# ISU-PAAL/DeepDFA

Measured on AMD Instinct MI355X. Metric: train_graphs_per_sec, higher is better.
Workload: dtype bf16; 1 GPU; model=DeepDFA-FlowGNN-GGNN(n_steps=5,D=128), global_batch=256, avg_nodes_per_graph=45, parallelism=dp1

## Files before the change

csrc/bindings.hip:

```cpp

#include <torch/extension.h>

#include <hip/hip_runtime.h>
#include <hip/hip_bf16.h>
#include <c10/hip/HIPStream.h>
#include <c10/util/accumulate.h>

#include <climits>

template <typename T>
void launch_embed4_fwd(const T*, const long*, T*, int, int, hipStream_t);
template <typename T, typename TO>
void launch_embed4_fwd2(const T*, const long*, TO*, int, int, hipStream_t);
template <typename T>
void launch_embed4_bwd(const T*, const long*, float*, long, int, hipStream_t);
template <typename T>
void launch_spmm_sum(const int*, const int*, const T*, T*, int, int, hipStream_t);
template <typename T>
void launch_gru_gates_fwd(const T*, const T*, const T*, T*, T*, T*, T*, long, int, hipStream_t);
template <typename T>
void launch_gru_gates_bwd(const T*, const T*, const T*, const T*, const T*, const T*, T*, T*, T*,
                          long, int, hipStream_t);
template <typename T>
void launch_attn_pool_fwd(const T*, const T*, const int*, T*, float*, int, int, hipStream_t);
template <typename T>
void launch_attn_pool_bwd(const T*, const T*, const float*, const int*, T*, T*, float*, int, int,
                          hipStream_t);
void launch_segment_max(const float*, const int*, float*, int, hipStream_t);
template <typename T>
void launch_gru_gates2_fwd(const T*, const T*, T*, T*, T*, T*, T*, long, int, hipStream_t);
template <typename T>
void launch_gru_gates2_bwd(const T*, const T*, const T*, const T*, const T*, const T*, T*, T*,
                           long, int, hipStream_t);
template <typename T>
void launch_colsum(const T*, float*, int, int, hipStream_t);
template <typename T>
void launch_spmm_sum_strided(const int*, const int*, const T*, T*, int, int, long,
                             hipStream_t);
void launch_gemm_bias2(const __hip_bfloat16*, const __hip_bfloat16*, const __hip_bfloat16*,
                       const __hip_bfloat16*, const __hip_bfloat16*, long,
                       const __hip_bfloat16*, long, __hip_bfloat16*, int, int, int, int,
                       hipStream_t, const int* = nullptr, const int* = nullptr, long = 0,
                       __hip_bfloat16* = nullptr);
bool launch_gates_gemm(const __hip_bfloat16*, const __hip_bfloat16*, const __hip_bfloat16*,
                       const __hip_bfloat16*, const __hip_bfloat16*, const __hip_bfloat16*,
                       const __hip_bfloat16*, __hip_bfloat16*, __hip_bfloat16*,
                       __hip_bfloat16*, int, int, hipStream_t);
void launch_gemm_bias(const __hip_bfloat16*, const __hip_bfloat16*, const __hip_bfloat16*,
                      const __hip_bfloat16*, const __hip_bfloat16*, __hip_bfloat16*, int, int,
                      int, int, hipStream_t);
void launch_wgrad(const __hip_bfloat16*, const __hip_bfloat16*, const __hip_bfloat16*, float*,
                  float*, int, int, int, int, hipStream_t, float* = nullptr,
                  float* = nullptr, float* = nullptr, float* = nullptr);
template <typename T>
void launch_layernorm_fwd(const T*, const float*, const float*, T*, float*, float*, long, int,
                          float, hipStream_t);
template <typename T>
void launch_layernorm_bwd(const T*, const T*, const float*, const float*, const float*, T*, long,
                          int, hipStream_t);
template <typename T>
void launch_layernorm_wgrad(const T*, const T*, const float*, const float*, float*, float*, long,
                            int, hipStream_t);
template <typename T>
void launch_bias_gelu_fwd(const T*, const float*, T*, long, int, hipStream_t);
template <typename T>
void launch_bias_gelu_bwd(const T*, const T*, const float*, T*, long, int, hipStream_t);
template <typename T>
void launch_softmax_mask_fwd(const T*, const int*, T*, T*, long, int, int, float, float,
                             unsigned long long, int, int, hipStream_t);
template <typename T>
void launch_rmsnorm_fwd(const T*, const float*, T*, float*, long, int, float, hipStream_t);
template <typename T>
void launch_rmsnorm_bwd(const T*, const T*, const float*, const float*, T*, long, int,
                        hipStream_t);
template <typename T>
void launch_rmsnorm_wgrad(const T*, const T*, const float*, float*, long, int, hipStream_t);
void launch_flash_fwd(const __hip_bfloat16*, const __hip_bfloat16*, const __hip_bfloat16*,
                      const int*, const float*, __hip_bfloat16*, float*, int, int, int, float,
                      int, unsigned, unsigned long long, long, long, hipStream_t);
void launch_flash_dterm(const __hip_bfloat16*, const __hip_bfloat16*, float*, int, int, int,
                        hipStream_t);
void launch_flash_dq(const __hip_bfloat16*, const __hip_bfloat16*, const __hip_bfloat16*,
                     const __hip_bfloat16*, const int*, const float*, const float*, const float*,
                     __hip_bfloat16*, float*, int, int, int, float, int, unsigned,
                     unsigned long long, long, long, long, hipStream_t);
void launch_wgrad2(const __hip_bfloat16*, const __hip_bfloat16*, float*, float*,
                   int, int, int, int, hipStream_t);
void launch_adamw_fused(float*, const float*, float*, float*, long, float, float, float, float,
                        float, const float*, const float*, int, void*, hipStream_t);
void launch_gemm2(const __hip_bfloat16*, const __hip_bfloat16*, const float*,
                  const __hip_bfloat16*, __hip_bfloat16*, int, int, int, hipStream_t);
void launch_flash_dkv(const __hip_bfloat16*, const __hip_bfloat16*, const __hip_bfloat16*,
                      const __hip_bfloat16*, const int*, const float*, const float*, const float*,
                      __hip_bfloat16*, __hip_bfloat16*, int, int, int, float, int, unsigned,
                      unsigned long long, long, long, long, hipStream_t);
template <typename T>
void launch_softmax_mask_bwd(const T*, const T*, T*, long, int, float, float,
                             unsigned long long, hipStream_t);
void launch_flash_received(const __hip_bfloat16*, const __hip_bfloat16*, const int*, const float*,
                           const float*, float*, int, int, int, float, int, long, long,
                           hipStream_t);
void dkv_prof_fetch(unsigned long long*);
void fwd_prof_fetch(unsigned long long*);
template <typename T>
void launch_dropout_add_fwd(const T*, const T*, T*, long, float, unsigned long long,
                            hipStream_t);
template <typename T>
void launch_dropout_add_bwd(const T*, T*, long, float, unsigned long long, hipStream_t);
template <typename T>
void launch_ln_res_dropout_fwd(const T*, const T*, const float*, const float*, T*, float*,
                               float*, long, int, float, float, unsigned long long, hipStream_t);
template <typename T>
void launch_ln_res_dropout_bwd(const T*, const T*, const T*, const float*, const float*,
                               const float*, T*, T*, T*, long, int, float,
                               unsigned long long, hipStream_t);
template <typename T>
void launch_ln_res_dropout_wgrad(const T*, const T*, const T*, const float*, const float*,
                                 float*, float*, long, int, float, unsigned long long,
                                 hipStream_t);
template <typename T>
void launch_embed_scatter(const T*, const long*, float*, long, int, long, hipStream_t);
void launch_relbias_wgrad(const float*, const int*, float*, long, int, int,
                          hipStream_t);
template <typename T>
void launch_relu_dropout_fwd(const T*, T*, long, float, unsigned long long, hipStream_t);
template <typename T>
void launch_relu_dropout_bwd(const T*, const T*, T*, long, float, unsigned long long,
                             hipStream_t);

#define CHECK_GPU(t) \
  TORCH_CHECK((t).is_cuda() && (t).is_contiguous(), #t " must be contiguous GPU tensor")

static hipStream_t cur_stream() {
  return c10::hip::getCurrentHIPStream().stream();
}

template <typename F>
void dispatch_float_bf16(const at::Tensor& t, const char* name, F&& f) {
  if (t.scalar_type() == at::kFloat) {
    f(float{});
  } else if (t.scalar_type() == at::kBFloat16) {
    f(__hip_bfloat16{});
  } else {
    TORCH_CHECK(false, name, ": unsupported dtype ", t.scalar_type());
  }
}

static at::Tensor acc_or_zeros(const c10::optional<at::Tensor>& out, at::IntArrayRef shape,
                               const at::TensorOptions& like, const char* name) {
  if (!out.has_value()) return at::zeros(shape, like.dtype(at::kFloat));
  TORCH_CHECK(out->is_cuda() && out->scalar_type() == at::kFloat && out->is_contiguous() &&
                  out->numel() == c10::multiply_integers(shape),
              name, ": accumulator must be a contiguous fp32 GPU tensor of ",
              c10::multiply_integers(shape), " elements");
  return *out;
}

template <typename T>
const T* ptr(const at::Tensor& t) {
  return reinterpret_cast<const T*>(t.data_ptr());
}
template <typename T>
T* mptr(at::Tensor& t) {
  return reinterpret_cast<T*>(t.data_ptr());
}

at::Tensor embed4_fwd(at::Tensor tables, at::Tensor idx, bool out_bf16 = false) {
  CHECK_GPU(tables);
// ... 169 lines not shown
  const bool acc = out_opt.has_value();
  auto out = acc_or_zeros(out_opt, {M, C}, A.options(), "wgrad");
  if (M % 128 == 0 && C % 128 == 0) {
    launch_wgrad2(ptr<bf16_t>(A), ptr<bf16_t>(B), out.data_ptr<float>(), nullptr,
                  K, M, C, acc ? 1 : 0, cur_stream());
    return out;
  }
  launch_wgrad(ptr<bf16_t>(A), ptr<bf16_t>(B), nullptr, out.data_ptr<float>(), nullptr,
               K, M, C, C, cur_stream());
  return out;
}

void launch_pack_gru_weights(const float*, const float*, const float*, const float*,
                             const float*, const float*, int, __hip_bfloat16*,
                             __hip_bfloat16*, __hip_bfloat16*, __hip_bfloat16*,
                             __hip_bfloat16*, __hip_bfloat16*, __hip_bfloat16*,
                             __hip_bfloat16*, hipStream_t);
void launch_gemm_gru(const __hip_bfloat16*, const __hip_bfloat16*, const __hip_bfloat16*,
                     const __hip_bfloat16*, const __hip_bfloat16*, __hip_bfloat16*,
                     __hip_bfloat16*, __hip_bfloat16*, __hip_bfloat16*, __hip_bfloat16*,
                     int, int, int, int, hipStream_t, const int* = nullptr,
                     const int* = nullptr, __hip_bfloat16* = nullptr);

void pack_gru_weights(at::Tensor W_e, at::Tensor b_e, at::Tensor W_ih, at::Tensor W_hh,
                      at::Tensor b_ih, at::Tensor b_hh, at::Tensor w_e16, at::Tensor b_e16,
                      at::Tensor Wcat, at::Tensor WcatT, at::Tensor b_cat, at::Tensor W_eT,
                      at::Tensor Wcat_perm, at::Tensor b_perm) {
  CHECK_GPU(W_e);
  const int H = W_e.size(0);
  TORCH_CHECK(W_e.scalar_type() == at::kFloat && W_ih.scalar_type() == at::kFloat,
              "pack_gru_weights reads fp32 master weights");
  TORCH_CHECK(Wcat.size(0) == 4 * H && Wcat.size(1) == 2 * H);
  launch_pack_gru_weights(W_e.data_ptr<float>(), b_e.data_ptr<float>(),
                          W_ih.data_ptr<float>(), W_hh.data_ptr<float>(),
                          b_ih.data_ptr<float>(), b_hh.data_ptr<float>(), H,
                          mptr<bf16_t>(w_e16), mptr<bf16_t>(b_e16), mptr<bf16_t>(Wcat),
                          mptr<bf16_t>(WcatT), mptr<bf16_t>(b_cat), mptr<bf16_t>(W_eT),
                          mptr<bf16_t>(Wcat_perm), mptr<bf16_t>(b_perm),
                          cur_stream());
}

std::vector<at::Tensor> ggnn_fused_fwd(at::Tensor indptr, at::Tensor indices, at::Tensor x,
                                       at::Tensor W_e, at::Tensor b_e, at::Tensor Wcat_perm,
                                       at::Tensor b_perm, long n_steps, bool fuse) {
  CHECK_GPU(x);
  TORCH_CHECK(x.scalar_type() == at::kBFloat16, "fused GGNN path is bf16");
  const long N = x.size(0);
  const long H = x.size(1);
  TORCH_CHECK(H % 64 == 0 && (4 * H) % 128 == 0, "H must suit the MFMA tile");
  TORCH_CHECK(Wcat_perm.size(0) == 4 * H && Wcat_perm.size(1) == 2 * H &&
              b_perm.numel() == 4 * H,
              "Wcat_perm/b_perm must be prebuilt (ops/flowgnn.py cache)");
  auto stream = cur_stream();
  const long S = n_steps;
  auto opts = x.options();
  auto HH = at::empty({S + 1, N, H}, opts);
  HH.select(0, 0).copy_(x);
  auto M = at::empty({S, N, H}, opts);
  auto R = at::empty({S, N, H}, opts);
  auto Z = at::empty({S, N, H}, opts);
  auto Nn = at::empty({S, N, H}, opts);
  auto HN = at::empty({S, N, H}, opts);
  auto wh = at::empty({N, H}, opts);
  const long NH = N * H;
  for (long s = 0; s < S; ++s) {
    const bf16_t* h = ptr<bf16_t>(HH) + s * NH;
    launch_gemm_bias(h, nullptr, ptr<bf16_t>(W_e), ptr<bf16_t>(b_e), nullptr, mptr<bf16_t>(wh),
                     N, H, H, H, stream);
    bf16_t* m = mptr<bf16_t>(M) + s * NH;
    if (!fuse)
      launch_spmm_sum<bf16_t>(indptr.data_ptr<int>(), indices.data_ptr<int>(), ptr<bf16_t>(wh),
                              m, N, H, stream);
    launch_gemm_gru(fuse ? ptr<bf16_t>(wh) : m, h, ptr<bf16_t>(Wcat_perm), ptr<bf16_t>(b_perm),
                    h, mptr<bf16_t>(HH) + (s + 1) * NH, mptr<bf16_t>(R) + s * NH,
                    mptr<bf16_t>(Z) + s * NH, mptr<bf16_t>(Nn) + s * NH,
                    mptr<bf16_t>(HN) + s * NH, N, 2 * H, H, H, stream,
                    fuse ? indptr.data_ptr<int>() : nullptr,
                    fuse ? indices.data_ptr<int>() : nullptr, fuse ? m : nullptr);
  }
  auto h_final = HH.select(0, S);
  return {h_final, HH, M, R, Z, Nn, HN};
}

std::vector<at::Tensor> ggnn_fused_bwd(at::Tensor grad_out, at::Tensor t_indptr,
                                       at::Tensor t_indices, at::Tensor x, at::Tensor W_eT,
                                       at::Tensor WcatT, at::Tensor HH,
                                       at::Tensor M, at::Tensor R, at::Tensor Z, at::Tensor Nn,
                                       at::Tensor HN, long n_steps,
                                       c10::optional<at::Tensor> out_we,
                                       c10::optional<at::Tensor> out_be,
                                       c10::optional<std::vector<at::Tensor>> gru_outs,
                                       bool fuse) {
  const long N = x.size(0);
  const long H = x.size(1);
  const long S = n_steps;
  const long NH = N * H;
  auto stream = cur_stream();
  TORCH_CHECK(WcatT.size(0) == 2 * H && WcatT.size(1) == 4 * H && W_eT.size(0) == H,
              "WcatT/W_eT must be prebuilt (ops/flowgnn.py cache)");
  auto opts = x.options();
  auto Ggicat = at::empty({S, N, 4 * H}, opts);
  auto Gwh = at::empty({S, N, H}, opts);
  auto go = grad_out.contiguous();
  auto grad_h = S > 0 ? at::empty({N, H}, opts) : go.clone();
  auto grad_hd = at::empty({N, H}, opts);
  auto grad_A = at::empty({N, 2 * H}, opts);
  for (long s = S - 1; s >= 0; --s) {
    const bf16_t* h_in = ptr<bf16_t>(HH) + s * NH;
    const bf16_t* g_in = (s == S - 1) ? ptr<bf16_t>(go) : ptr<bf16_t>(grad_h);
    auto ggic = Ggicat.select(0, s);
    auto gwh = Gwh.select(0, s);
    if (!fuse ||
        !launch_gates_gemm(g_in, h_in, ptr<bf16_t>(R) + s * NH, ptr<bf16_t>(Z) + s * NH,
                           ptr<bf16_t>(Nn) + s * NH, ptr<bf16_t>(HN) + s * NH,
                           ptr<bf16_t>(WcatT), mptr<bf16_t>(ggic), mptr<bf16_t>(grad_hd),
                           mptr<bf16_t>(grad_A), N, H, stream)) {
      launch_gru_gates2_bwd<bf16_t>(g_in, h_in, ptr<bf16_t>(R) + s * NH,
                                    ptr<bf16_t>(Z) + s * NH, ptr<bf16_t>(Nn) + s * NH,
                                    ptr<bf16_t>(HN) + s * NH, mptr<bf16_t>(ggic),
                                    mptr<bf16_t>(grad_hd), NH, H, stream);
      launch_gemm_bias(ptr<bf16_t>(ggic), nullptr, ptr<bf16_t>(WcatT), nullptr, nullptr,
                       mptr<bf16_t>(grad_A), N, 4 * H, 4 * H, 2 * H, stream);
    }
    if (fuse) {
      launch_gemm_bias2(ptr<bf16_t>(grad_A), nullptr, ptr<bf16_t>(W_eT), nullptr,
                        ptr<bf16_t>(grad_hd), H, ptr<bf16_t>(grad_A) + H, 2 * H,
                        mptr<bf16_t>(grad_h), N, H, H, H, stream,
                        t_indptr.data_ptr<int>(), t_indices.data_ptr<int>(), 2 * H,
                        mptr<bf16_t>(gwh));
    } else {
      launch_spmm_sum_strided<bf16_t>(t_indptr.data_ptr<int>(), t_indices.data_ptr<int>(),
                                      ptr<bf16_t>(grad_A), mptr<bf16_t>(gwh), N, H,
                                      2 * H, stream);
      launch_gemm_bias2(ptr<bf16_t>(gwh), nullptr, ptr<bf16_t>(W_eT), nullptr,
                        ptr<bf16_t>(grad_hd), H, ptr<bf16_t>(grad_A) + H, 2 * H,
                        mptr<bf16_t>(grad_h), N, H, H, H, stream);
    }
  }
  auto A_g = Ggicat.view({S * N, 4 * H});
  const bool gru_direct = gru_outs.has_value();
  at::Tensor gWcat, cs4;
  if (gru_direct) {
    TORCH_CHECK(gru_outs->size() == 4, "gru_outs = [gW_ih, gW_hh, gb_ih, gb_hh]");
    for (auto& t : *gru_outs)
      TORCH_CHECK(t.is_cuda() && t.scalar_type() == at::kFloat && t.is_contiguous());
    TORCH_CHECK((*gru_outs)[0].numel() == 3 * H * H &&
                (*gru_outs)[1].numel() == 3 * H * H &&
                (*gru_outs)[2].numel() == 3 * H && (*gru_outs)[3].numel() == 3 * H);
  } else {
    gWcat = at::zeros({4 * H, 2 * H}, opts.dtype(at::kFloat));
    cs4 = at::zeros({4 * H}, opts.dtype(at::kFloat));
  }
  if (gru_direct)
    launch_wgrad(ptr<bf16_t>(A_g), ptr<bf16_t>(M), ptr<bf16_t>(HH), nullptr, nullptr,
                 S * N, 4 * H, 2 * H, H, stream, (*gru_outs)[0].data_ptr<float>(),
                 (*gru_outs)[1].data_ptr<float>(), (*gru_outs)[2].data_ptr<float>(),
                 (*gru_outs)[3].data_ptr<float>());
  else
    launch_wgrad(ptr<bf16_t>(A_g), ptr<bf16_t>(M), ptr<bf16_t>(HH), gWcat.data_ptr<float>(),
                 cs4.data_ptr<float>(), S * N, 4 * H, 2 * H, H, stream);
  auto A_w = Gwh.view({S * N, H});
  const bool acc_we = out_we.has_value();
  TORCH_CHECK(out_be.has_value() == acc_we, "ggnn_fused_bwd: out_we and out_be go together");
  auto gW_e = acc_or_zeros(out_we, {H, H}, opts, "ggnn_fused_bwd out_we");
  auto cs_e = acc_or_zeros(out_be, {H}, opts, "ggnn_fused_bwd out_be");
  if (H % 128 == 0)
    launch_wgrad2(ptr<bf16_t>(A_w), ptr<bf16_t>(HH), gW_e.data_ptr<float>(),
                  cs_e.data_ptr<float>(), S * N, H, H, acc_we ? 1 : 0, stream);
  else
    launch_wgrad(ptr<bf16_t>(A_w), ptr<bf16_t>(HH), nullptr, gW_e.data_ptr<float>(),
                 cs_e.data_ptr<float>(), S * N, H, H, H, stream);
  if (gru_direct) {
    auto none = at::empty({0}, opts.dtype(at::kFloat));
    return {grad_h, gW_e, cs_e, none, none, none, none};
  }
  auto gW_ih = gWcat.narrow(0, 0, 3 * H).narrow(1, 0, H);
  auto gW_hh = at::cat({gWcat.narrow(0, 0, 2 * H).narrow(1, H, H),
                        gWcat.narrow(0, 3 * H, H).narrow(1, H, H)});
  auto gb_ih = cs4.narrow(0, 0, 3 * H).contiguous();
  auto gb_hh = at::cat({cs4.narrow(0, 0, 2 * H), cs4.narrow(0, 3 * H, H)});
  return {grad_h, gW_e, cs_e, gW_ih, gW_hh, gb_ih, gb_hh};
}

std::vector<at::Tensor> gru_gates2_fwd(at::Tensor gicat, at::Tensor h) {
  CHECK_GPU(gicat);
  CHECK_GPU(h);
  const long N = h.size(0);
  const int H = h.size(1);
  auto h_new = at::empty_like(h);
  auto r = at::empty_like(h);
  auto z = at::empty_like(h);
  auto n = at::empty_like(h);
  auto hn = at::empty_like(h);
  dispatch_float_bf16(h, "gru_gates2_fwd", [&](auto tag) {
    using T = decltype(tag);
    launch_gru_gates2_fwd<T>(ptr<T>(gicat), ptr<T>(h), mptr<T>(h_new), mptr<T>(r), mptr<T>(z),
                             mptr<T>(n), mptr<T>(hn), N * H, H, cur_stream());
  });
  return {h_new, r, z, n, hn};
}

std::vector<at::Tensor> gru_gates2_bwd(at::Tensor grad_h_new, at::Tensor h, at::Tensor r,
                                       at::Tensor z, at::Tensor n, at::Tensor hn) {
  CHECK_GPU(grad_h_new);
  CHECK_GPU(h);
  const long N = h.size(0);
  const int H = h.size(1);
  for (const at::Tensor* t : {&grad_h_new, &r, &z, &n, &hn})
    TORCH_CHECK(t->is_cuda() && t->is_contiguous() && t->sizes() == h.sizes() &&
                    t->scalar_type() == h.scalar_type(),
                "gru_gates2_bwd: operands must match h");
  auto grad_gicat = at::empty({N, 4 * H}, h.options());
  auto grad_h = at::empty_like(h);
  dispatch_float_bf16(h, "gru_gates2_bwd", [&](auto tag) {
    using T = decltype(tag);
    launch_gru_gates2_bwd<T>(ptr<T>(grad_h_new), ptr<T>(h), ptr<T>(r), ptr<T>(z), ptr<T>(n),
                             ptr<T>(hn), mptr<T>(grad_gicat), mptr<T>(grad_h), N * H, H,
                             cur_stream());
  });
  return {grad_gicat, grad_h};
// ... 904 lines not shown
      launch_ln_res_dropout_bwd<T>(ptr<T>(dy), ptr<T>(h), ptr<T>(res),
                                   gamma.data_ptr<float>(), mean.data_ptr<float>(),
                                   rstd.data_ptr<float>(), mptr<T>(dz), mptr<T>(dh),
                                   mptr<T>(z), N, D, (float)p, (unsigned long long)seed,
                                   cur_stream());
    });
    return std::vector<at::Tensor>{dz, dh, z};
  });
  m.def("ln_res_dropout_wgrad", [](at::Tensor dy, at::Tensor h, at::Tensor res,
                                   at::Tensor mean, at::Tensor rstd, double p,
                                   int64_t seed) {
    tk_lead("ln_res_dropout_wgrad", dy);
    const int D = dy.size(-1);
    const long N = dy.numel() / D;
    tk_arg("ln_res_dropout_wgrad", "h", h, dy, dy.scalar_type(), dy.sizes());
    tk_arg("ln_res_dropout_wgrad", "res", res, dy, dy.scalar_type(), dy.sizes());
    tk_arg("ln_res_dropout_wgrad", "mean", mean, dy, at::kFloat, {N});
    tk_arg("ln_res_dropout_wgrad", "rstd", rstd, dy, at::kFloat, {N});
    auto dgamma = at::zeros({(long)D}, dy.options().dtype(at::kFloat));
    auto dbeta = at::zeros({(long)D}, dy.options().dtype(at::kFloat));
    dispatch_float_bf16(dy, "ln_res_dropout_wgrad", [&](auto tag) {
      using T = decltype(tag);
      launch_ln_res_dropout_wgrad<T>(ptr<T>(dy), ptr<T>(h), ptr<T>(res),
                                     mean.data_ptr<float>(), rstd.data_ptr<float>(),
                                     dgamma.data_ptr<float>(), dbeta.data_ptr<float>(), N,
                                     D, (float)p, (unsigned long long)seed, cur_stream());
    });
    return std::vector<at::Tensor>{dgamma, dbeta};
  });
  m.def("embed_scatter", [](at::Tensor dY, at::Tensor idx, long num_rows, long padding_idx,
                            c10::optional<at::Tensor> out_opt) {
    tk_lead("embed_scatter", dY);
    const int D = dY.size(-1);
    const long N = dY.numel() / D;
    TORCH_CHECK(idx.numel() == N, "embed_scatter: idx must have one entry per row of dY");
    tk_arg("embed_scatter", "idx", idx, dY, at::kLong, idx.sizes());
    auto dW = acc_or_zeros(out_opt, {num_rows, (long)D}, dY.options(), "embed_scatter");
    dispatch_float_bf16(dY, "embed_scatter", [&](auto tag) {
      using T = decltype(tag);
      launch_embed_scatter<T>(ptr<T>(dY), idx.data_ptr<long>(),
                              dW.data_ptr<float>(), N, D, padding_idx,
                              cur_stream());
    });
    return dW;
  }, pybind11::arg("dY"), pybind11::arg("idx"), pybind11::arg("num_rows"),
     pybind11::arg("padding_idx"), pybind11::arg("out") = pybind11::none());
  m.def("fwd_prof", []() {
    auto t = torch::zeros({8}, torch::dtype(torch::kLong));
    fwd_prof_fetch(reinterpret_cast<unsigned long long*>(t.data_ptr<long>()));
    return t;
  });
  m.def("dkv_prof", []() {
    auto t = torch::zeros({8}, torch::dtype(torch::kLong));
    dkv_prof_fetch(reinterpret_cast<unsigned long long*>(t.data_ptr<long>()));
    return t;
  });
  m.def("gemm2", &gemm2);
  m.def("adamw_fused", &adamw_fused, pybind11::arg("p"), pybind11::arg("g"),
        pybind11::arg("m"), pybind11::arg("v"), pybind11::arg("lr"),
        pybind11::arg("beta1"), pybind11::arg("beta2"), pybind11::arg("eps"),
        pybind11::arg("weight_decay"), pybind11::arg("step"),
        pybind11::arg("gclip") = pybind11::none(),
        pybind11::arg("l2_mode") = false,
        pybind11::arg("p16") = pybind11::none());
  m.def("softmax_mask_bwd", &softmax_mask_bwd);
  m.def("node_head_fwd", &node_head_fwd, pybind11::arg("h"), pybind11::arg("fe"),
        pybind11::arg("W1"), pybind11::arg("W2"), pybind11::arg("b1"), pybind11::arg("b2"),
        pybind11::arg("w3"), pybind11::arg("b3"), pybind11::arg("save") = true,
        pybind11::arg("tile_rows") = 0);
  m.def("node_head_bwd", &node_head_bwd, pybind11::arg("dlogits"), pybind11::arg("H1"),
        pybind11::arg("H2"), pybind11::arg("W1T"), pybind11::arg("W2T"), pybind11::arg("w3"),
        pybind11::arg("out_w3") = pybind11::none(), pybind11::arg("out_b3") = pybind11::none(),
        pybind11::arg("tile_rows") = 0);
  m.def("node_head_tile_rows", [](int64_t N, int64_t tile) {
    return node_head_tile_rows((int)N, (int)tile);
  }, pybind11::arg("N"), pybind11::arg("tile_rows") = 0);
  m.def("ggnn_fused_bwd", &ggnn_fused_bwd, pybind11::arg("grad_out"),
        pybind11::arg("t_indptr"), pybind11::arg("t_indices"), pybind11::arg("x"),
        pybind11::arg("W_eT"), pybind11::arg("WcatT"), pybind11::arg("HH"),
        pybind11::arg("M"), pybind11::arg("R"), pybind11::arg("Z"), pybind11::arg("Nn"),
        pybind11::arg("HN"), pybind11::arg("n_steps"),
        pybind11::arg("out_we") = pybind11::none(),
        pybind11::arg("out_be") = pybind11::none(),
        pybind11::arg("gru_outs") = pybind11::none(), pybind11::arg("fuse") = true);
}
```

csrc/wgrad2.hip:

```cpp

#include <hip/hip_runtime.h>
#include <hip/hip_bf16.h>
#include <cstdlib>

#define WAVE 64
#define WBM 128
#define WBC 128
#define WBK 64

using bf16 = __hip_bfloat16;
using bf16x8 = __attribute__((ext_vector_type(8))) __bf16;
using f32x4 = __attribute__((ext_vector_type(4))) float;
using uint4v = __attribute__((ext_vector_type(4))) unsigned int;

__device__ __forceinline__ void w2_load(const bf16* __restrict__ src, long ld,
                                        int k0, int col0, int tid,
                                        uint4v regs[4], int k_lim) {
  const int kr = tid >> 4;
  const int c8 = (tid & 15) * 8;
  if (k0 + 64 <= k_lim) {
#pragma unroll
    for (int p = 0; p < 4; ++p)
      regs[p] = *reinterpret_cast<const uint4v*>(
          src + (long)(k0 + kr + 16 * p) * ld + col0 + c8);
  } else {
#pragma unroll
    for (int p = 0; p < 4; ++p) {
      const int k = k0 + kr + 16 * p;
      regs[p] = {};
      if (k < k_lim)
        regs[p] = *reinterpret_cast<const uint4v*>(src + (long)k * ld + col0 + c8);
    }
  }
}

__global__ __launch_bounds__(256) void wgrad2_kernel(
    const bf16* __restrict__ A, const bf16* __restrict__ B,
    float* __restrict__ out, float* __restrict__ csum, int K, int M, int C,
    int kchunk, int zsplit) {
  extern __shared__ __attribute__((aligned(16))) char smem[];
#define W2_SUBB 144
#define W2_SUB(kb, cb) (((kb)*8 + (cb)) * W2_SUBB)
#define W2_TILEB (16 * 8 * W2_SUBB)
#define A_LDS(i) (smem + (i) * (2 * W2_TILEB))
#define B_LDS(i) (smem + W2_TILEB + (i) * (2 * W2_TILEB))

using bf16x4v = __attribute__((ext_vector_type(4))) __bf16;
typedef __attribute__((address_space(3))) bf16x4v lds_bf16x4;
  const int m0 = blockIdx.x * WBM;
  const int c0 = blockIdx.y * WBC;
  const int k_begin = blockIdx.z * kchunk;
  const int k_end = min(K, k_begin + kchunk);
  const int tid = threadIdx.x;
  const int lane = tid & (WAVE - 1);
  const int wid = tid >> 6;
  const int wm = wid >> 1;
  const int wc = wid & 1;

  f32x4 acc[4][4] = {};
  float cs_acc = 0.f;
  const bool do_csum = (csum != nullptr) && (blockIdx.y == 0) && (tid < 128);

  auto write_nat = [&](char* lds, const uint4v regs[4]) {
    const int kr = tid >> 4;
    const int cb = (tid & 15) >> 1;
    const int halfb = ((tid & 15) & 1) * 16;
#pragma unroll
    for (int p = 0; p < 4; ++p) {
      const int k = kr + 16 * p;
      *reinterpret_cast<uint4v*>(lds + W2_SUB(k >> 2, cb) + (k & 3) * 32 +
                                 halfb) = regs[p];
    }
  };

  uint4v a_regs[4], b_regs[4];
  w2_load(A, M, k_begin, m0, tid, a_regs, k_end);
  w2_load(B, C, k_begin, c0, tid, b_regs, k_end);
  write_nat(A_LDS(0), a_regs);
  write_nat(B_LDS(0), b_regs);
  __syncthreads();

  int cur = 0;
  for (int k0 = k_begin; k0 < k_end; k0 += WBK) {
    const bool has_next = (k0 + WBK) < k_end;
    if (has_next) {
      w2_load(A, M, k0 + WBK, m0, tid, a_regs, k_end);
      w2_load(B, C, k0 + WBK, c0, tid, b_regs, k_end);
    }
    if (do_csum) {
      const int klim = min(WBK, k_end - k0);
      const int cb = tid >> 4, cc = (tid & 15) * 2;
#pragma unroll 8
      for (int k = 0; k < klim; ++k)
        cs_acc += __bfloat162float(*reinterpret_cast<const __bf16*>(
            A_LDS(cur) + W2_SUB(k >> 2, cb) + (k & 3) * 32 + cc));
    }
#pragma unroll 1
    for (int ks = 0; ks < 2; ++ks) {
      const int kb0 = ks * 8 + (lane >> 4) * 2;
      const int slot = (lane & 15) * 8;
      bf16x8 a_frag[4], b_frag[4];
#pragma unroll
      for (int f = 0; f < 4; ++f) {
        const int cba = wm * 4 + f;
        const int cbb = wc * 4 + f;
        bf16x4v* af = reinterpret_cast<bf16x4v*>(&a_frag[f]);
        bf16x4v* bf = reinterpret_cast<bf16x4v*>(&b_frag[f]);
        af[0] = __builtin_amdgcn_ds_read_tr16_b64_v4bf16(
            (lds_bf16x4*)(A_LDS(cur) + W2_SUB(kb0, cba) + slot));
        af[1] = __builtin_amdgcn_ds_read_tr16_b64_v4bf16(
            (lds_bf16x4*)(A_LDS(cur) + W2_SUB(kb0 + 1, cba) + slot));
        bf[0] = __builtin_amdgcn_ds_read_tr16_b64_v4bf16(
            (lds_bf16x4*)(B_LDS(cur) + W2_SUB(kb0, cbb) + slot));
        bf[1] = __builtin_amdgcn_ds_read_tr16_b64_v4bf16(
            (lds_bf16x4*)(B_LDS(cur) + W2_SUB(kb0 + 1, cbb) + slot));
      }
      __builtin_amdgcn_s_setprio(1);
#pragma unroll
      for (int fm = 0; fm < 4; ++fm)
#pragma unroll
        for (int fc = 0; fc < 4; ++fc)
          acc[fm][fc] = __builtin_amdgcn_mfma_f32_16x16x32_bf16(
              a_frag[fm], b_frag[fc], acc[fm][fc], 0, 0, 0);
      __builtin_amdgcn_s_setprio(0);
    }
    __syncthreads();
    if (has_next) {
      write_nat(A_LDS(cur ^ 1), a_regs);
      write_nat(B_LDS(cur ^ 1), b_regs);
    }
    __syncthreads();
    cur ^= 1;
  }

#undef A_LDS
#undef B_LDS
  if (do_csum) {
    const int m = m0 + (tid >> 4) * 16 + (tid & 15);
    if (m < M) atomicAdd(csum + m, cs_acc);
  }
#pragma unroll
  for (int fm = 0; fm < 4; ++fm) {
    const int m_base = m0 + wm * 64 + fm * 16 + (lane >> 4) * 4;
#pragma unroll
    for (int fc = 0; fc < 4; ++fc) {
      const int c = c0 + wc * 64 + fc * 16 + (lane & 15);
#pragma unroll
      for (int i = 0; i < 4; ++i) {
        if (zsplit == 1)
          out[(long)(m_base + i) * C + c] = acc[fm][fc][i];
        else
          atomicAdd(out + (long)(m_base + i) * C + c, acc[fm][fc][i]);
      }
    }
  }
}

void launch_wgrad2(const bf16* A, const bf16* B, float* out, float* csum,
                   int K, int M, int C, int accumulate, hipStream_t stream) {
  const int tiles = (M / WBM) * (C / WBC);
  int kfloor = 768;
  if (const char* e = getenv("DFA_WG2_KFLOOR")) kfloor = atoi(e);
  int zsplit = max(1, 512 / tiles);
  int kchunk = (K + zsplit - 1) / zsplit;
  kchunk = ((kchunk + WBK - 1) / WBK) * WBK;
  if (kchunk < kfloor) kchunk = min(((K + WBK - 1) / WBK) * WBK, kfloor);
  zsplit = (K + kchunk - 1) / kchunk;
  const dim3 grid(M / WBM, C / WBC, zsplit);
  const int zarg = accumulate ? max(zsplit, 2) : zsplit;
  hipLaunchKernelGGL(wgrad2_kernel, grid, dim3(256), 73728, stream, A, B, out,
                     csum, K, M, C, kchunk, zarg);
}
```

setup.py:

```python

import os

from setuptools import setup

os.environ.setdefault("PYTORCH_ROCM_ARCH", "gfx950")

from torch.utils.cpp_extension import BuildExtension, CUDAExtension

HERE = os.path.dirname(os.path.abspath(__file__))

ext = CUDAExtension(
    name="deepdfa_amd._C",
    sources=[
        "csrc/bindings.hip",
        "csrc/flowgnn_kernels.hip",
        "csrc/gemm_bias.hip",
        "csrc/wgrad.hip",
        "csrc/transformer_kernels.hip",
        "csrc/flash_attn.hip",
        "csrc/gemm_bf16.hip",
        "csrc/wgrad2.hip",
        "csrc/adamw.hip",
        "csrc/lmhead_ce.hip",
        "csrc/node_head.hip",
        "csrc/graph_head.hip",
    ],
    depends=["csrc/mfma_tile.h", "csrc/gru_gate_bwd.h"],
    extra_compile_args={
        "cxx": ["-O3", "-std=c++17"],
        "nvcc": ["-O3", "-std=c++17"],
    },
)

setup(
    name="deepdfa_amd",
    version="0.1.0",
    packages=["deepdfa_amd"],
    ext_modules=[ext],
    cmdclass={"build_ext": BuildExtension.with_options(no_python_abi_suffix=False)},
)
```

Baseline: 493,700 graphs/s.

## Fuse GGNN GRU and edge-linear weight gradients into one split-K MFMA kernel

Adds a single kernel that computes all GGNN weight gradients (the GRU input and hidden weights, their biases, and the edge-linear W_e and b_e) in one launch. It uses seven 128x128 tiles, a split-K over all S*N rows and XCD-aware block ordering, and folds the bias column sums into the operand loads. This replaces the separate wgrad and wgrad2 launches and their reductions, and it is enabled by default through a new fused_wgrad flag. The change relies on float atomics for split-K accumulation, which makes results nondeterministic and adds atomic traffic, and it only applies when H=128.

```diff
diff --git a/csrc/bindings.hip b/csrc/bindings.hip
--- a/csrc/bindings.hip
+++ b/csrc/bindings.hip
@@ -84,6 +84,10 @@
                      const __hip_bfloat16*, const int*, const float*, const float*, const float*,
                      __hip_bfloat16*, float*, int, int, int, float, int, unsigned,
                      unsigned long long, long, long, long, hipStream_t);
+void launch_ggnn_wgrad(const __hip_bfloat16*, const __hip_bfloat16*, const __hip_bfloat16*,
+                       const __hip_bfloat16*, float*, float*, float*, float*, float*, float*,
+                       int, int, int, int, hipStream_t);
+int ggnn_wgrad_kchunk(int, int);
 void launch_wgrad2(const __hip_bfloat16*, const __hip_bfloat16*, float*, float*,
                    int, int, int, int, hipStream_t);
 void launch_adamw_fused(float*, const float*, float*, float*, long, float, float, float, float,
@@ -419,6 +423,71 @@
   return {h_final, HH, M, R, Z, Nn, HN};
 }
 
+static std::vector<at::Tensor> ggnn_wgrad_run(const at::Tensor& Ggicat, const at::Tensor& M,
+                                              const at::Tensor& HH, const at::Tensor& Gwh,
+                                              long K, long H,
+                                              const c10::optional<at::Tensor>& out_we,
+                                              const c10::optional<at::Tensor>& out_be,
+                                              const c10::optional<std::vector<at::Tensor>>& gru_outs,
+                                              long kchunk = 0, long lds_epi = -1,
+                                              bool two_launches = false) {
+  TORCH_CHECK(H == 128, "ggnn_wgrad is written for H = 128");
+  TORCH_CHECK(out_be.has_value() == out_we.has_value(),
+              "ggnn_wgrad: out_we and out_be go together");
+  auto opts = Ggicat.options();
+  const bool gru_direct = gru_outs.has_value();
+  if (gru_direct)
+    TORCH_CHECK(gru_outs->size() == 4, "gru_outs = [gW_ih, gW_hh, gb_ih, gb_hh]");
+  auto pick = [&](int i) {
+    return gru_direct ? c10::optional<at::Tensor>((*gru_outs)[i]) : c10::nullopt;
+  };
+  auto gW_ih = acc_or_zeros(pick(0), {3 * H, H}, opts, "ggnn_wgrad gW_ih");
+  auto gW_hh = acc_or_zeros(pick(1), {3 * H, H}, opts, "ggnn_wgrad gW_hh");
+  auto gb_ih = acc_or_zeros(pick(2), {3 * H}, opts, "ggnn_wgrad gb_ih");
+  auto gb_hh = acc_or_zeros(pick(3), {3 * H}, opts, "ggnn_wgrad gb_hh");
+  auto gW_e = acc_or_zeros(out_we, {H, H}, opts, "ggnn_wgrad out_we");
+  auto gb_e = acc_or_zeros(out_be, {H}, opts, "ggnn_wgrad out_be");
+  if (two_launches) {
+    launch_wgrad(ptr<bf16_t>(Ggicat), ptr<bf16_t>(M), ptr<bf16_t>(HH), nullptr, nullptr, K,
+                 4 * H, 2 * H, H, cur_stream(), gW_ih.data_ptr<float>(),
+                 gW_hh.data_ptr<float>(), gb_ih.data_ptr<float>(), gb_hh.data_ptr<float>());
+    launch_wgrad2(ptr<bf16_t>(Gwh), ptr<bf16_t>(HH), gW_e.data_ptr<float>(),
+                  gb_e.data_ptr<float>(), K, H, H, 1, cur_stream());
+    return {gW_ih, gW_hh, gb_ih, gb_hh, gW_e, gb_e};
+  }
+  launch_ggnn_wgrad(ptr<bf16_t>(Ggicat), ptr<bf16_t>(Gwh), ptr<bf16_t>(M), ptr<bf16_t>(HH),
+                    gW_ih.data_ptr<float>(), gW_hh.data_ptr<float>(), gW_e.data_ptr<float>(),
+                    gb_ih.data_ptr<float>(), gb_hh.data_ptr<float>(), gb_e.data_ptr<float>(),
+                    (int)K, gru_direct ? 1 : 0, (int)kchunk, (int)lds_epi, cur_stream());
+  if (!gru_direct) gb_hh.narrow(0, 0, 2 * H).copy_(gb_ih.narrow(0, 0, 2 * H));
+  return {gW_ih, gW_hh, gb_ih, gb_hh, gW_e, gb_e};
+}
+
+std::vector<at::Tensor> ggnn_wgrad(at::Tensor Ggicat, at::Tensor M, at::Tensor HH,
+                                   at::Tensor Gwh, long S,
+                                   c10::optional<at::Tensor> out_we,
+                                   c10::optional<at::Tensor> out_be,
+                                   c10::optional<std::vector<at::Tensor>> gru_outs,
+                                   long kchunk, long lds_epi, bool two_launches) {
+  CHECK_GPU(Ggicat);
+  CHECK_GPU(M);
+  CHECK_GPU(HH);
+  CHECK_GPU(Gwh);
+  for (const at::Tensor* t : {&Ggicat, &M, &HH, &Gwh})
+    TORCH_CHECK(t->scalar_type() == at::kBFloat16 && t->dim() == 3, "ggnn_wgrad: (S, N, cols) bf16");
+  const long N = M.size(1);
+  const long H = M.size(2);
+  TORCH_CHECK(S >= 0 && Ggicat.size(0) >= S && M.size(0) >= S && HH.size(0) >= S &&
+                  Gwh.size(0) >= S,
+              "ggnn_wgrad: fewer than S slabs");
+  TORCH_CHECK(Ggicat.size(1) == N && HH.size(1) == N && Gwh.size(1) == N &&
+                  Ggicat.size(2) == 4 * H && HH.size(2) == H && Gwh.size(2) == H,
+              "ggnn_wgrad: operand shapes disagree");
+  TORCH_CHECK(S * N < (1L << 31), "ggnn_wgrad: S*N must fit an int");
+  return ggnn_wgrad_run(Ggicat, M, HH, Gwh, S * N, H, out_we, out_be, gru_outs, kchunk,
+                        lds_epi, two_launches);
+}
+
 std::vector<at::Tensor> ggnn_fused_bwd(at::Tensor grad_out, at::Tensor t_indptr,
                                        at::Tensor t_indices, at::Tensor x, at::Tensor W_eT,
                                        at::Tensor WcatT, at::Tensor HH,
@@ -427,7 +496,7 @@
                                        c10::optional<at::Tensor> out_we,
                                        c10::optional<at::Tensor> out_be,
                                        c10::optional<std::vector<at::Tensor>> gru_outs,
-                                       bool fuse) {
+                                       bool fuse, bool fused_wgrad) {
   const long N = x.size(0);
   const long H = x.size(1);
   const long S = n_steps;
@@ -473,6 +542,14 @@
                         ptr<bf16_t>(grad_hd), H, ptr<bf16_t>(grad_A) + H, 2 * H,
                         mptr<bf16_t>(grad_h), N, H, H, H, stream);
     }
+  }
+  if (fused_wgrad && H == 128) {
+    auto g = ggnn_wgrad_run(Ggicat, M, HH, Gwh, S * N, H, out_we, out_be, gru_outs);
+    if (gru_outs.has_value()) {
+      auto none = at::empty({0}, opts.dtype(at::kFloat));
+      return {grad_h, g[4], g[5], none, none, none, none};
+    }
+    return {grad_h, g[4], g[5], g[0], g[1], g[2], g[3]};
   }
   auto A_g = Ggicat.view({S * N, 4 * H});
   const bool gru_direct = gru_outs.has_value();
@@ -1543,5 +1620,14 @@
         pybind11::arg("HN"), pybind11::arg("n_steps"),
         pybind11::arg("out_we") = pybind11::none(),
         pybind11::arg("out_be") = pybind11::none(),
-        pybind11::arg("gru_outs") = pybind11::none(), pybind11::arg("fuse") = true);
-}
+        pybind11::arg("gru_outs") = pybind11::none(), pybind11::arg("fuse") = true,
+        pybind11::arg("fused_wgrad") = true);
+  m.def("ggnn_wgrad", &ggnn_wgrad, pybind11::arg("Ggicat"), pybind11::arg("M"),
+        pybind11::arg("HH"), pybind11::arg("Gwh"), pybind11::arg("S"),
+        pybind11::arg("out_we") = pybind11::none(), pybind11::arg("out_be") = pybind11::none(),
+        pybind11::arg("gru_outs") = pybind11::none(), pybind11::arg("kchunk") = 0,
+        pybind11::arg("lds_epi") = -1, pybind11::arg("two_launches") = false);
+  m.def("ggnn_wgrad_kchunk", [](int64_t K, int64_t kchunk) {
+    return ggnn_wgrad_kchunk((int)K, (int)kchunk);
+  }, pybind11::arg("K"), pybind11::arg("kchunk") = 0);
+}
diff --git a/csrc/ggnn_wgrad.hip b/csrc/ggnn_wgrad.hip
--- /dev/null
+++ b/csrc/ggnn_wgrad.hip
@@ -0,0 +1,203 @@
+
+#include <hip/hip_runtime.h>
+
+#include "wgrad_tr16.h"
+
+#define GW_H 128
+#define GW_TILES 7
+#define GW_XCD 8
+#define GW_LDS (4 * W2_TILEB)
+#define GW_EPI_LD 132
+
+struct GgnnWgradArgs {
+  const bf16* ggicat;
+  const bf16* gwh;
+  const bf16* m;
+  const bf16* hh;
+  float* w_ih;
+  float* w_hh;
+  float* w_e;
+  float* b_ih;
+  float* b_hh;
+  float* b_e;
+  int K;
+  int kchunk;
+  int zsplit;
+  int b_hh_rz;
+};
+
+__device__ __forceinline__ void gw_colsum(const uint4v regs[4], float cs[8]) {
+#pragma unroll
+  for (int p = 0; p < 4; ++p)
+#pragma unroll
+    for (int j = 0; j < 4; ++j) {
+      cs[2 * j] += __uint_as_float(regs[p][j] << 16);
+      cs[2 * j + 1] += __uint_as_float(regs[p][j] & 0xffff0000u);
+    }
+}
+
+template <bool LDS_EPI>
+__global__ __launch_bounds__(256, 2) void ggnn_wgrad_kernel(GgnnWgradArgs p) {
+  extern __shared__ __attribute__((aligned(16))) char smem[];
+#define A_LDS(i) (smem + (i) * (2 * W2_TILEB))
+#define B_LDS(i) (smem + W2_TILEB + (i) * (2 * W2_TILEB))
+
+  const int x = blockIdx.x % GW_XCD;
+  const int g = blockIdx.x / GW_XCD;
+  const int tile = g % GW_TILES;
+  const int chunk = (g / GW_TILES) * GW_XCD + x;
+  if (chunk >= p.zsplit) return;
+
+  const bool we = tile == 6;
+  const int ablk = tile < 3 ? tile : (tile == 5 ? 3 : tile - 3);
+  const bf16* A = we ? p.gwh : p.ggicat;
+  const long lda = we ? GW_H : 4 * GW_H;
+  const int acol = we ? 0 : ablk * GW_H;
+  const bf16* B = tile < 3 ? p.m : p.hh;
+  float* out = we ? p.w_e
+                  : (tile < 3 ? p.w_ih + tile * GW_H * GW_H
+                              : p.w_hh + (tile - 3) * GW_H * GW_H);
+  float* cs1 = nullptr;
+  float* cs2 = nullptr;
+  if (tile < 3) cs1 = p.b_ih + tile * GW_H;
+  if (tile < 2 && p.b_hh_rz) cs2 = p.b_hh + tile * GW_H;
+  if (tile == 5) cs1 = p.b_hh + 2 * GW_H;
+  if (we) cs1 = p.b_e;
+  const bool owner = cs1 != nullptr;
+
+  const int k_begin = chunk * p.kchunk;
+  const int k_end = min(p.K, k_begin + p.kchunk);
+  const int tid = threadIdx.x;
+  const int lane = tid & (WAVE - 1);
+  const int wid = tid >> 6;
+  const int wm = wid >> 1;
+  const int wc = wid & 1;
+
+  f32x4 acc[4][4] = {};
+  float cs[8] = {};
+
+  uint4v a_regs[4], b_regs[4];
+  w2_load(A, lda, k_begin, acol, tid, a_regs, k_end);
+  w2_load(B, GW_H, k_begin, 0, tid, b_regs, k_end);
+  w2_write_nat(A_LDS(0), a_regs, tid);
+  w2_write_nat(B_LDS(0), b_regs, tid);
+  if (owner) gw_colsum(a_regs, cs);
+  __syncthreads();
+
+  int cur = 0;
+  for (int k0 = k_begin; k0 < k_end; k0 += WBK) {
+    const bool has_next = (k0 + WBK) < k_end;
+    if (has_next) {
+      w2_load(A, lda, k0 + WBK, acol, tid, a_regs, k_end);
+      w2_load(B, GW_H, k0 + WBK, 0, tid, b_regs, k_end);
+    }
+#pragma unroll 1
+    for (int ks = 0; ks < 2; ++ks)
+      w2_mfma_step(A_LDS(cur), B_LDS(cur), ks, lane, wm, wc, acc);
+    __syncthreads();
+    if (has_next) {
+      w2_write_nat(A_LDS(cur ^ 1), a_regs, tid);
+      w2_write_nat(B_LDS(cur ^ 1), b_regs, tid);
+      if (owner) gw_colsum(a_regs, cs);
+    }
+    __syncthreads();
+    cur ^= 1;
+  }
+#undef A_LDS
+#undef B_LDS
+
+  float* fs = reinterpret_cast<float*>(smem);
+  if (owner) {
+    float* row = fs + (tid >> 4) * GW_H + (tid & 15) * 8;
+    *reinterpret_cast<f32x4*>(row) = f32x4{cs[0], cs[1], cs[2], cs[3]};
+    *reinterpret_cast<f32x4*>(row + 4) = f32x4{cs[4], cs[5], cs[6], cs[7]};
+    __syncthreads();
+    if (tid < GW_H) {
+      float s = 0.f;
+#pragma unroll
+      for (int r = 0; r < 16; ++r) s += fs[r * GW_H + tid];
+      atomicAdd(cs1 + tid, s);
+      if (cs2 != nullptr) atomicAdd(cs2 + tid, s);
+    }
+    if (LDS_EPI) __syncthreads();
+  }
+
+  if (LDS_EPI) {
+#pragma unroll
+    for (int fm = 0; fm < 4; ++fm) {
+      const int m_base = wm * 64 + fm * 16 + (lane >> 4) * 4;
+#pragma unroll
+      for (int fc = 0; fc < 4; ++fc) {
+        const int c = wc * 64 + fc * 16 + (lane & 15);
+#pragma unroll
+        for (int i = 0; i < 4; ++i) fs[(m_base + i) * GW_EPI_LD + c] = acc[fm][fc][i];
+      }
+    }
+    __syncthreads();
+#pragma unroll 8
+    for (int r = 0; r < 32; ++r) {
+      const int m = wid * 32 + r;
+      atomicAdd(out + m * GW_H + lane, fs[m * GW_EPI_LD + lane]);
+      atomicAdd(out + m * GW_H + 64 + lane, fs[m * GW_EPI_LD + 64 + lane]);
+    }
+  } else {
+#pragma unroll
+    for (int fm = 0; fm < 4; ++fm) {
+      const int m_base = wm * 64 + fm * 16 + (lane >> 4) * 4;
+#pragma unroll
+      for (int fc = 0; fc < 4; ++fc) {
+        const int c = wc * 64 + fc * 16 + (lane & 15);
+#pragma unroll
+        for (int i = 0; i < 4; ++i)
+          atomicAdd(out + (m_base + i) * GW_H + c, acc[fm][fc][i]);
+      }
+    }
+  }
+}
+
+#define GW_ZTARGET 56
+#define GW_KCHUNK_MIN 768
+#define GW_LDS_EPI_DEFAULT 1
+
+int ggnn_wgrad_kchunk(int K, int kchunk) {
+  if (kchunk <= 0) kchunk = max((K + GW_ZTARGET - 1) / GW_ZTARGET, GW_KCHUNK_MIN);
+  return ((kchunk + WBK - 1) / WBK) * WBK;
+}
+
+void launch_ggnn_wgrad(const bf16* ggicat, const bf16* gwh, const bf16* m, const bf16* hh,
+                       float* w_ih, float* w_hh, float* w_e, float* b_ih, float* b_hh,
+                       float* b_e, int K, int b_hh_rz, int kchunk, int lds_epi,
+                       hipStream_t stream) {
+  if (K <= 0) return;
+  static const bool raised = [] {
+    return hipFuncSetAttribute(reinterpret_cast<const void*>(&ggnn_wgrad_kernel<true>),
+                               hipFuncAttributeMaxDynamicSharedMemorySize,
+                               GW_LDS) == hipSuccess &&
+           hipFuncSetAttribute(reinterpret_cast<const void*>(&ggnn_wgrad_kernel<false>),
+                               hipFuncAttributeMaxDynamicSharedMemorySize,
+                               GW_LDS) == hipSuccess;
+  }();
+  (void)raised;
+  GgnnWgradArgs p;
+  p.ggicat = ggicat;
+  p.gwh = gwh;
+  p.m = m;
+  p.hh = hh;
+  p.w_ih = w_ih;
+  p.w_hh = w_hh;
+  p.w_e = w_e;
+  p.b_ih = b_ih;
+  p.b_hh = b_hh;
+  p.b_e = b_e;
+  p.K = K;
+  p.kchunk = ggnn_wgrad_kchunk(K, kchunk);
+  p.zsplit = (K + p.kchunk - 1) / p.kchunk;
+  p.b_hh_rz = b_hh_rz;
+  const int groups = (p.zsplit + GW_XCD - 1) / GW_XCD;
+  const dim3 grid(groups * GW_TILES * GW_XCD);
+  if (lds_epi < 0) lds_epi = GW_LDS_EPI_DEFAULT;
+  if (lds_epi)
+    hipLaunchKernelGGL(ggnn_wgrad_kernel<true>, grid, dim3(256), GW_LDS, stream, p);
+  else
+    hipLaunchKernelGGL(ggnn_wgrad_kernel<false>, grid, dim3(256), GW_LDS, stream, p);
+}
diff --git a/csrc/wgrad2.hip b/csrc/wgrad2.hip
--- a/csrc/wgrad2.hip
+++ b/csrc/wgrad2.hip
@@ -1,52 +1,18 @@
+
+#include <cstdlib>
 
 #include <hip/hip_runtime.h>
-#include <hip/hip_bf16.h>
-#include <cstdlib>
 
-#define WAVE 64
-#define WBM 128
-#define WBC 128
-#define WBK 64
-
-using bf16 = __hip_bfloat16;
-using bf16x8 = __attribute__((ext_vector_type(8))) __bf16;
-using f32x4 = __attribute__((ext_vector_type(4))) float;
-using uint4v = __attribute__((ext_vector_type(4))) unsigned int;
-
-__device__ __forceinline__ void w2_load(const bf16* __restrict__ src, long ld,
-                                        int k0, int col0, int tid,
-                                        uint4v regs[4], int k_lim) {
-  const int kr = tid >> 4;
-  const int c8 = (tid & 15) * 8;
-  if (k0 + 64 <= k_lim) {
-#pragma unroll
-    for (int p = 0; p < 4; ++p)
-      regs[p] = *reinterpret_cast<const uint4v*>(
-          src + (long)(k0 + kr + 16 * p) * ld + col0 + c8);
-  } else {
-#pragma unroll
-    for (int p = 0; p < 4; ++p) {
-      const int k = k0 + kr + 16 * p;
-      regs[p] = {};
-      if (k < k_lim)
-        regs[p] = *reinterpret_cast<const uint4v*>(src + (long)k * ld + col0 + c8);
-    }
-  }
-}
+#include "wgrad_tr16.h"
 
 __global__ __launch_bounds__(256) void wgrad2_kernel(
     const bf16* __restrict__ A, const bf16* __restrict__ B,
     float* __restrict__ out, float* __restrict__ csum, int K, int M, int C,
     int kchunk, int zsplit) {
   extern __shared__ __attribute__((aligned(16))) char smem[];
-#define W2_SUBB 144
-#define W2_SUB(kb, cb) (((kb)*8 + (cb)) * W2_SUBB)
-#define W2_TILEB (16 * 8 * W2_SUBB)
 #define A_LDS(i) (smem + (i) * (2 * W2_TILEB))
 #define B_LDS(i) (smem + W2_TILEB + (i) * (2 * W2_TILEB))
 
-using bf16x4v = __attribute__((ext_vector_type(4))) __bf16;
-typedef __attribute__((address_space(3))) bf16x4v lds_bf16x4;
   const int m0 = blockIdx.x * WBM;
   const int c0 = blockIdx.y * WBC;
   const int k_begin = blockIdx.z * kchunk;
@@ -61,17 +27,7 @@
   float cs_acc = 0.f;
   const bool do_csum = (csum != nullptr) && (blockIdx.y == 0) && (tid < 128);
 
-  auto write_nat = [&](char* lds, const uint4v regs[4]) {
-    const int kr = tid >> 4;
-    const int cb = (tid & 15) >> 1;
-    const int halfb = ((tid & 15) & 1) * 16;
-#pragma unroll
-    for (int p = 0; p < 4; ++p) {
-      const int k = kr + 16 * p;
-      *reinterpret_cast<uint4v*>(lds + W2_SUB(k >> 2, cb) + (k & 3) * 32 +
-                                 halfb) = regs[p];
-    }
-  };
+  auto write_nat = [&](char* lds, const uint4v regs[4]) { w2_write_nat(lds, regs, tid); };
 
   uint4v a_regs[4], b_regs[4];
   w2_load(A, M, k_begin, m0, tid, a_regs, k_end);
@@ -97,32 +53,7 @@
     }
 #pragma unroll 1
     for (int ks = 0; ks < 2; ++ks) {
-      const int kb0 = ks * 8 + (lane >> 4) * 2;
-      const int slot = (lane & 15) * 8;
-      bf16x8 a_frag[4], b_frag[4];
-#pragma unroll
-      for (int f = 0; f < 4; ++f) {
-        const int cba = wm * 4 + f;
-        const int cbb = wc * 4 + f;
-        bf16x4v* af = reinterpret_cast<bf16x4v*>(&a_frag[f]);
-        bf16x4v* bf = reinterpret_cast<bf16x4v*>(&b_frag[f]);
-        af[0] = __builtin_amdgcn_ds_read_tr16_b64_v4bf16(
-            (lds_bf16x4*)(A_LDS(cur) + W2_SUB(kb0, cba) + slot));
-        af[1] = __builtin_amdgcn_ds_read_tr16_b64_v4bf16(
-            (lds_bf16x4*)(A_LDS(cur) + W2_SUB(kb0 + 1, cba) + slot));
-        bf[0] = __builtin_amdgcn_ds_read_tr16_b64_v4bf16(
-            (lds_bf16x4*)(B_LDS(cur) + W2_SUB(kb0, cbb) + slot));
-        bf[1] = __builtin_amdgcn_ds_read_tr16_b64_v4bf16(
-            (lds_bf16x4*)(B_LDS(cur) + W2_SUB(kb0 + 1, cbb) + slot));
-      }
-      __builtin_amdgcn_s_setprio(1);
-#pragma unroll
-      for (int fm = 0; fm < 4; ++fm)
-#pragma unroll
-        for (int fc = 0; fc < 4; ++fc)
-          acc[fm][fc] = __builtin_amdgcn_mfma_f32_16x16x32_bf16(
-              a_frag[fm], b_frag[fc], acc[fm][fc], 0, 0, 0);
-      __builtin_amdgcn_s_setprio(0);
+      w2_mfma_step(A_LDS(cur), B_LDS(cur), ks, lane, wm, wc, acc);
     }
     __syncthreads();
     if (has_next) {
diff --git a/csrc/wgrad_tr16.h b/csrc/wgrad_tr16.h
--- /dev/null
+++ b/csrc/wgrad_tr16.h
@@ -0,0 +1,82 @@
+#pragma once
+
+#include <hip/hip_runtime.h>
+#include <hip/hip_bf16.h>
+
+#define WAVE 64
+#define WBM 128
+#define WBC 128
+#define WBK 64
+
+using bf16 = __hip_bfloat16;
+using bf16x8 = __attribute__((ext_vector_type(8))) __bf16;
+using f32x4 = __attribute__((ext_vector_type(4))) float;
+using uint4v = __attribute__((ext_vector_type(4))) unsigned int;
+using bf16x4v = __attribute__((ext_vector_type(4))) __bf16;
+typedef __attribute__((address_space(3))) bf16x4v lds_bf16x4;
+
+#define W2_SUBB 144
+#define W2_SUB(kb, cb) (((kb)*8 + (cb)) * W2_SUBB)
+#define W2_TILEB (16 * 8 * W2_SUBB)
+
+__device__ __forceinline__ void w2_load(const bf16* __restrict__ src, long ld,
+                                        int k0, int col0, int tid,
+                                        uint4v regs[4], int k_lim) {
+  const int kr = tid >> 4;
+  const int c8 = (tid & 15) * 8;
+  if (k0 + 64 <= k_lim) {
+#pragma unroll
+    for (int p = 0; p < 4; ++p)
+      regs[p] = *reinterpret_cast<const uint4v*>(
+          src + (long)(k0 + kr + 16 * p) * ld + col0 + c8);
+  } else {
+#pragma unroll
+    for (int p = 0; p < 4; ++p) {
+      const int k = k0 + kr + 16 * p;
+      regs[p] = {};
+      if (k < k_lim)
+        regs[p] = *reinterpret_cast<const uint4v*>(src + (long)k * ld + col0 + c8);
+    }
+  }
+}
+
+__device__ __forceinline__ void w2_write_nat(char* lds, const uint4v regs[4], int tid) {
+  const int kr = tid >> 4;
+  const int cb = (tid & 15) >> 1;
+  const int halfb = ((tid & 15) & 1) * 16;
+#pragma unroll
+  for (int p = 0; p < 4; ++p) {
+    const int k = kr + 16 * p;
+    *reinterpret_cast<uint4v*>(lds + W2_SUB(k >> 2, cb) + (k & 3) * 32 + halfb) = regs[p];
+  }
+}
+
+__device__ __forceinline__ void w2_mfma_step(const char* a_lds, const char* b_lds, int ks,
+                                             int lane, int wm, int wc, f32x4 acc[4][4]) {
+  const int kb0 = ks * 8 + (lane >> 4) * 2;
+  const int slot = (lane & 15) * 8;
+  bf16x8 a_frag[4], b_frag[4];
+#pragma unroll
+  for (int f = 0; f < 4; ++f) {
+    const int cba = wm * 4 + f;
+    const int cbb = wc * 4 + f;
+    bf16x4v* af = reinterpret_cast<bf16x4v*>(&a_frag[f]);
+    bf16x4v* bf = reinterpret_cast<bf16x4v*>(&b_frag[f]);
+    af[0] = __builtin_amdgcn_ds_read_tr16_b64_v4bf16(
+        (lds_bf16x4*)(a_lds + W2_SUB(kb0, cba) + slot));
+    af[1] = __builtin_amdgcn_ds_read_tr16_b64_v4bf16(
+        (lds_bf16x4*)(a_lds + W2_SUB(kb0 + 1, cba) + slot));
+    bf[0] = __builtin_amdgcn_ds_read_tr16_b64_v4bf16(
+        (lds_bf16x4*)(b_lds + W2_SUB(kb0, cbb) + slot));
+    bf[1] = __builtin_amdgcn_ds_read_tr16_b64_v4bf16(
+        (lds_bf16x4*)(b_lds + W2_SUB(kb0 + 1, cbb) + slot));
+  }
+  __builtin_amdgcn_s_setprio(1);
+#pragma unroll
+  for (int fm = 0; fm < 4; ++fm)
+#pragma unroll
+    for (int fc = 0; fc < 4; ++fc)
+      acc[fm][fc] = __builtin_amdgcn_mfma_f32_16x16x32_bf16(
+          a_frag[fm], b_frag[fc], acc[fm][fc], 0, 0, 0);
+  __builtin_amdgcn_s_setprio(0);
+}
diff --git a/setup.py b/setup.py
--- a/setup.py
+++ b/setup.py
@@ -20,12 +20,13 @@
         "csrc/flash_attn.hip",
         "csrc/gemm_bf16.hip",
         "csrc/wgrad2.hip",
+        "csrc/ggnn_wgrad.hip",
         "csrc/adamw.hip",
         "csrc/lmhead_ce.hip",
         "csrc/node_head.hip",
         "csrc/graph_head.hip",
     ],
-    depends=["csrc/mfma_tile.h", "csrc/gru_gate_bwd.h"],
+    depends=["csrc/mfma_tile.h", "csrc/gru_gate_bwd.h", "csrc/wgrad_tr16.h"],
     extra_compile_args={
         "cxx": ["-O3", "-std=c++17"],
         "nvcc": ["-O3", "-std=c++17"],
```

New measurement: 562,700 graphs/s, median of 6. +14.0%, better.
